# nemo110110/modify-sift-gpu

Hardware: AMD Instinct MI355X
Metric: SIFT images/sec at 1080p (features/sec alongside), 1/2/4/8 MI355X (higher is better)
Workload: dtype f32

## Files before the change

### include/sgpu.h

```cpp
#ifndef SGPU_H
#define SGPU_H
#include <stddef.h>
#include <stdint.h>

#ifdef __cplusplus
extern "C" {
#endif

#define SGPU_OK 0
#define SGPU_EINVAL (-1)
#define SGPU_ENODEV (-2)
#define SGPU_ENOMEM (-3)
#define SGPU_ERANGE (-4)

typedef struct sgpu_options {
    float filter_width_factor;
    float descriptor_window_factor;
    float orientation_window_factor;
    float orientation_gaussian_factor;
    float dog_threshold;
    float edge_threshold;
    int subpixel;
    int max_orientation;
    int fixed_orientation;
// ... 134 lines not shown
#define SGPU_DEBUG_FULL_COLUMNS 128
#define SGPU_DEBUG_DESC_DUAL 256
#define SGPU_DEBUG_ORIENT_WAVE 512
#define SGPU_DEBUG_GAUSS_TILE_ALWAYS 1024
#define SGPU_DEBUG_MATCH_REGSTAGE 2048
#define SGPU_DEBUG_PYR_SERIAL 4096
#define SGPU_DEBUG_GAUSS_LONG_BANDS 8192
#define SGPU_DEBUG_DUO_ALWAYS 16384
#define SGPU_DEBUG_DUO_OFF 32768
#define SGPU_DEBUG_GAUSS_TILE_OFF 65536
#define SGPU_DEBUG_DESC_WIDE_OFF 131072
#define SGPU_DEBUG_DESC_WIDE_ALWAYS 262144
#define SGPU_DEBUG_EXTREMA_TILE_OFF 524288

int sgpu_debug_set_flags(sgpu_ctx* ctx, int flags);
#define SGPU_TRIO_OFF 0
#define SGPU_TRIO_ON 1
#define SGPU_TRIO_ALWAYS 2
#define SGPU_PAIRS_FRONT 0
#define SGPU_PAIRS_END 1
int sgpu_debug_set_schedule(sgpu_ctx* ctx, int trio, int pairs);
#define SGPU_DUO_STRIPS_RULE 0
#define SGPU_DUO_STRIPS_WAVE 1
#define SGPU_DUO_STRIPS_COOP 2
int sgpu_debug_set_duo_strips(sgpu_ctx* ctx, int mode);
int sgpu_debug_set_match_prune(sgpu_ctx* ctx, int on);
int sgpu_debug_match_plan_stats(const sgpu_ctx* ctx, long long out[4]);
#define SGPU_PLAN_ENTRY_INTS 7
#define SGPU_PLAN_LEVEL 0
#define SGPU_PLAN_TILE 1
// ... 17 lines not shown
```

### modify-sift-gpu_amd/csrc/sgpu_capi.cpp

```cpp
#include <dlfcn.h>
#include <hip/hip_runtime.h>
#include <rccl/rccl.h>

#include <algorithm>
#include <cmath>
#include <cstdio>
#include <cstdlib>
#include <atomic>
#include <cstring>
#include <string>
#include <vector>

#include "../../include/sgpu.h"
#include "sift_kernels.h"
#include "sift_match_plan.h"
#include "sift_params.h"
#include "sift_pyramid_plan.h"

namespace {

#ifndef SGK_WIDE_DESC_MAX
#define SGK_WIDE_DESC_MAX 8192
#endif

// ... 81 lines not shown
struct sgpu_ctx {
    int device = 0;
    hipStream_t stream = nullptr;
    sgpu_options opt{};
    sgp::Schedule sched{};
    sgp::InputPlan plan{};
    int debug_flags = 0;
    bool multi_stream = false;
    bool duo_on = false;
    bool duo_wide = false;
    bool duo_u8 = false;
    int trio_mode = SGPU_TRIO_OFF;
    int duo_plan = SGK_DUO_PLAN;
    int duo_strips = SGPU_DUO_STRIPS_RULE;
    size_t wide_desc_max = SGK_WIDE_DESC_MAX;
    bool unit_input = true;
    bool tile_duo = false;
    int tile_mb = SGK_TILE_MB;
    int env_flags = 0;
    struct HostOut {
        float* keys = nullptr;
        float* desc = nullptr;
        int cap = 0;
        bool armed = false, active = false, done = false;
    } host_out;
    bool stage_timing = true;
    bool streaming = false;
    std::string err;
    int batch = 0, w = 0, h = 0, nparts = 0;
    std::vector<sgp::Octave> oct;
    size_t staged_bytes = 0;
    std::vector<int64_t> img_off;
    Part part[kMaxParts];
    DevBuf input, all_keys, all_desc, gray, pre;
// ... 193 lines not shown
    ctx->device = device;
    if (hipSetDevice(device) != hipSuccess ||
        hipStreamCreateWithFlags(&ctx->stream, hipStreamNonBlocking) != hipSuccess) {
        delete ctx;
        return SGPU_ENODEV;
    }
    for (int i = 0; i <= T_N; i++) (void)hipEventCreate(&ctx->ev[i]);
    {
        Part* p = ctx->part;
        bool ok = part_streams(p[0], PS_MAIN) == SGPU_OK && part_streams(p[0], PS_OCT) == SGPU_OK &&
                  hipStreamCreateWithFlags(&ctx->h2d, hipStreamNonBlocking) == hipSuccess &&
                  hipStreamCreateWithFlags(&ctx->d2h, hipStreamNonBlocking) == hipSuccess &&
                  part_streams(p[0], PS_LO) == SGPU_OK && part_streams(p[1], PS_OCT) == SGPU_OK &&
                  part_streams(p[2], PS_MAIN) == SGPU_OK && part_streams(p[2], PS_LO) == SGPU_OK &&
                  part_streams(p[1], PS_MAIN) == SGPU_OK && part_streams(p[1], PS_LO) == SGPU_OK;
        for (int i = 0; ok && i < 2; i++)
            ok = hipEventCreateWithFlags(&ctx->up_ev[i], hipEventDisableTiming) == hipSuccess &&
                 hipEventCreateWithFlags(&ctx->down_ev[i], hipEventDisableTiming) == hipSuccess;
        if (!ok) {
            sgpu_ctx_destroy(ctx);
            return SGPU_ENODEV;
        }
    }
    if (const char* ev = getenv("SGPU_EXACT_DESCRIPTOR"))
        if (ev[0] == '1') ctx->debug_flags |= SGPU_DEBUG_EXACT_DESCRIPTOR;
    if (const char* ev = getenv("SGPU_GAUSS")) {
        if (!strcmp(ev, "block")) ctx->debug_flags |= SGPU_DEBUG_GAUSS_BLOCK;
    }
    if (const char* ev = getenv("SGPU_DUO")) {
        if (!strcmp(ev, "off")) ctx->debug_flags |= SGPU_DEBUG_DUO_OFF;
// ... 22 lines not shown
    }
    if (const char* ev = getenv("SGPU_STREAMS")) ctx->multi_stream = !strcmp(ev, "multi");
    if (const char* ev = getenv("SGPU_MATCH"))
        if (!strcmp(ev, "reg")) ctx->debug_flags |= SGPU_DEBUG_MATCH_REGSTAGE;
    if (const char* ev = getenv("SGPU_DESC")) {
        if (!strcmp(ev, "dual")) ctx->debug_flags |= SGPU_DEBUG_DESC_DUAL;
        if (!strcmp(ev, "narrow")) ctx->debug_flags |= SGPU_DEBUG_DESC_WIDE_OFF;
        if (!strcmp(ev, "wide")) ctx->debug_flags |= SGPU_DEBUG_DESC_WIDE_ALWAYS;
    }
    if (const char* ev = getenv("SGPU_GAUSS_TILE")) {
        if (!strcmp(ev, "off")) ctx->debug_flags |= SGPU_DEBUG_GAUSS_TILE_OFF;
        if (!strcmp(ev, "always")) ctx->debug_flags |= SGPU_DEBUG_GAUSS_TILE_ALWAYS;
    }
    if (const char* ev = getenv("SGPU_WIDE_DESC_MAX"))
        if (atoll(ev) >= 0) ctx->wide_desc_max = (size_t)atoll(ev);
    if (const char* ev = getenv("SGPU_EXTREMA")) {
        if (!strcmp(ev, "wave")) ctx->debug_flags |= SGPU_DEBUG_EXTREMA_TILE_OFF;
    }
    if (const char* ev = getenv("SGPU_TILE_DUO"))
        ctx->tile_duo = !strcmp(ev, "on");
    if (const char* ev = getenv("SGPU_MATCH_PRUNE"))
        ctx->match_prune = strcmp(ev, "off") != 0;
    if (const char* ev = getenv("SGPU_GAUSS_TILE_MB"))
        if (atoi(ev) >= 0) ctx->tile_mb = atoi(ev);
    ctx->env_flags = ctx->debug_flags;
    int rc = sgpu_ctx_set_options(ctx, opt);
    if (rc != SGPU_OK) {
        sgpu_ctx_destroy(ctx);
        return rc;
    }
    *out = ctx;
    return SGPU_OK;
}
// ... 84 lines not shown
    fp.origin_offset = O.lowe_origin ? 0.0f : 0.5f;
    fp.octave_min = ctx->plan.octave_min + ctx->plan.ds;

    const size_t sum_px = (size_t)goff / (size_t)std::max(1, nlev) / (size_t)n;
    pt.cand_cap = (ctx->debug_flags & SGPU_DEBUG_TINY_CAP)
                      ? std::max<size_t>(pt.cand_cap, 64)
                      : std::max(pt.cand_cap, std::max<size_t>(1024, sum_px / 256 * n));
    const size_t nc = pt.cand_cap, ne_cap = 2 * nc;
    ALLOCCHK(ctx, pt.pyr.ensure((size_t)goff * sizeof(float) + 256));
    ALLOCCHK(ctx, pt.mask.ensure((size_t)moff * sizeof(uint32_t)));
    ALLOCCHK(ctx, pt.row_count.ensure((size_t)pt.total_rows * sizeof(uint32_t)));
    ALLOCCHK(ctx, pt.row_base.ensure(((size_t)pt.total_rows + 1) * sizeof(uint32_t)));
    ALLOCCHK(ctx, pt.img_off_dev.ensure((size_t)(n + 2) * sizeof(int64_t)));
    ALLOCCHK(ctx, pt.cand.ensure(nc * sizeof(float4)));
    ALLOCCHK(ctx, pt.info.ensure(nc * sizeof(int2)));
    ALLOCCHK(ctx, pt.ocount.ensure(nc * sizeof(uint32_t)));
    ALLOCCHK(ctx, pt.eoff.ensure((nc + 1) * sizeof(uint32_t)));
    ALLOCCHK(ctx, pt.feat.ensure(ne_cap * sizeof(float4)));
    ALLOCCHK(ctx, pt.feat_info.ensure(ne_cap * sizeof(int2)));
    ALLOCCHK(ctx, pt.keys.ensure(ne_cap * sizeof(float4)));
    if (O.descriptors) ALLOCCHK(ctx, pt.desc.ensure(ne_cap * 128 * sizeof(float)));
    ALLOCCHK(ctx, pt.scan_tmp.ensure((sgk::scan_tmp_words(std::max<size_t>(nc, pt.total_rows)) + 16) * 4));
    if (pt.h_read_n < (size_t)n + 2) {
        if (pt.h_read) (void)hipHostFree(pt.h_read);
        pt.h_read = nullptr;
        g_allocs++;
        ALLOCCHK(ctx, hipHostMalloc((void**)&pt.h_read, ((size_t)n + 2) * sizeof(int64_t)));
        pt.h_read_n = (size_t)n + 2;
    }
    return SGPU_OK;
}
// ... 58 lines not shown
            op.dst = lvl0 + k * od.level_stride;
            op.dst_img_stride = npx;
            op.w = od.wa;
            op.h = od.h;
            op.batch = n;
            op.ds_dst = dk ? ds : nullptr;
            op.ds_w = dk ? dsw : 0;
            op.ds_h = dk ? dsh : 0;
            op.ds_img_stride = dk ? ds_stride : 0;
            if (o == 0 && k == 0 && pt.one_stream) {
                op.zero.p[0] = pt.row_count.as<uint32_t>();
                op.zero.n[0] = (size_t)pt.total_rows;
                op.zero.p[1] = pt.mask.as<uint32_t>();
                op.zero.n[1] = (size_t)pt.mask_words;
                op.zero.p[2] = pt.ocount.as<uint32_t>();
                op.zero.n[2] = pt.cand_cap;
            }
            pt.levels.push_back(sgpyr::LevelDesc{o, k, op.fw, op.w, op.h, op.batch, dk,
                                                 op.src_u8 != nullptr,
                                                 (op.zero.n[0] | op.zero.n[1] | op.zero.n[2]) != 0});
        }
    }
    pt.gauss_filters = (int)pt.ops.size();
    return SGPU_OK;
}

struct OpSupport {
    const sgk::LevelOp* op;
    bool tile(int i) const { return sgk::gauss_tile_supported(op[i]); }
    bool tile_duo(int i, int j) const { return sgk::gauss_tile_duo_supported(op[i], op[j]); }
    bool duo(int i, int j) const { return sgk::gauss_duo_supported(op[i], op[j]); }
// ... 101 lines not shown
    if (O.feature_count_threshold > 0)
        HIPCHK(ctx, sgk::launch_limit_rows(pt.row_count.as<uint32_t>(), fp,
                                           O.feature_count_threshold, O.truncate_method, st));
    HIPCHK(ctx, rec(7, st));
    HIPCHK(ctx, sgk::launch_scan(pt.row_count.as<uint32_t>(), pt.row_base.as<uint32_t>(),
                                 pt.total_rows, pt.scan_tmp.as<uint32_t>(), st));
    HIPCHK(ctx, rec(2, st));

    if (!pt.one_stream) {
        st = pt.stream_lo;
        HIPCHK(ctx, hipStreamWaitEvent(st, pt.ev[2], 0));
    }
    if (wait_lo) HIPCHK(ctx, hipStreamWaitEvent(st, wait_lo, 0));
    const uint32_t* n_cand_dev = pt.row_base.as<uint32_t>() + pt.total_rows;
    if (!pt.one_stream)
        HIPCHK(ctx, sgk::launch_zero(pt.ocount.as<uint32_t>(), nc, nullptr, 0, nullptr, 0, st));
    const int cand_grid = (int)std::min(nc, pt.cand_hint ? pt.cand_hint : nc);
    const bool ori_wave = (ctx->debug_flags & SGPU_DEBUG_ORIENT_WAVE) ||
                          (pt.cand_hint > 0 && pt.cand_hint <= kWaveOrientationMax);
    const int feat_grid = (int)std::min(ne_cap, pt.feat_hint ? pt.feat_hint : ne_cap);
    const bool desc_wide = !(ctx->debug_flags & SGPU_DEBUG_DESC_WIDE_OFF) &&
                           ((ctx->debug_flags & SGPU_DEBUG_DESC_WIDE_ALWAYS) ||
                            (pt.feat_hint > 0 && pt.feat_hint <= ctx->wide_desc_max));
    HIPCHK(ctx, sgk::launch_orientation(pyr, pt.mask.as<uint32_t>(), pt.row_base.as<uint32_t>(),
                                        pt.total_rows, n_cand_dev, (int)nc, cand_grid, fp,
                                        pt.cand.as<float4>(), pt.info.as<int2>(),
                                        pt.ocount.as<uint32_t>(), st, ori_wave));
    if (O.feature_count_threshold > 0 && fp.num_orientation >= 2)
        HIPCHK(ctx, sgk::launch_limit_oriented(pt.ocount.as<uint32_t>(), pt.row_base.as<uint32_t>(),
                                               fp, O.feature_count_threshold, O.truncate_method,
                                               (uint32_t)nc, st));
    HIPCHK(ctx, rec(3, st));
    const uint32_t* n_feat_dev = pt.eoff.as<uint32_t>() + nc;
    sgk::ImageOffsetsArgs io;
    io.row_base = pt.row_base.as<uint32_t>();
    io.batch = n;
    io.rows_per_image = fp.rows_per_image;
    io.total_rows = pt.total_rows;
    io.off = pt.img_off_dev.as<int64_t>();
    HIPCHK(ctx, sgk::launch_scan(pt.ocount.as<uint32_t>(), pt.eoff.as<uint32_t>(), nc,
                                 pt.scan_tmp.as<uint32_t>(), st));
    HIPCHK(ctx, sgk::launch_expand(pt.cand.as<float4>(), pt.info.as<int2>(),
// ... 7 lines not shown
    const bool host_in_desc = pt.copied_out && O.descriptors && desc_wide && !exact_desc && !dual_desc;
    sgk::HostCopy hcopy;
    if (host_in_desc) {
        hcopy.keys = pt.keys.as<float4>();
        hcopy.rec = pt.img_off_dev.as<int64_t>();
        hcopy.rec_n = n + 2;
        hcopy.cap = (uint32_t)ctx->host_out.cap;
        hcopy.hkeys = reinterpret_cast<float4*>(ctx->host_out.keys);
        hcopy.hdesc = ctx->host_out.desc;
        hcopy.hrec = pt.h_read;
    }
    if (O.descriptors)
        HIPCHK(ctx, sgk::launch_descriptor(pyr, pt.feat.as<float4>(), pt.feat_info.as<int2>(),
                                           n_feat_dev, feat_grid, fp, pt.desc.as<float>(), st,
                                           nullptr, false, exact_desc, dual_desc, desc_wide,
                                           host_in_desc ? &hcopy : nullptr));
    HIPCHK(ctx, rec(5, st));
    if (pt.copied_out && !host_in_desc)
        HIPCHK(ctx, sgk::launch_copy_out(pt.keys.as<float4>(), O.descriptors ? pt.desc.as<float>() : nullptr,
                                         n_feat_dev, ctx->host_out.cap, pt.img_off_dev.as<int64_t>(),
                                         n + 2, ctx->host_out.keys,
                                         O.descriptors ? ctx->host_out.desc : nullptr, pt.h_read, st));
    return SGPU_OK;
}

static int enqueue_readback(sgpu_ctx* ctx, Part& pt) {
    hipStream_t st = pt.one_stream ? pt.stream : pt.stream_lo;
    if (!pt.copied_out)
        HIPCHK(ctx, hipMemcpyAsync(pt.h_read, pt.img_off_dev.p, (size_t)(pt.n + 2) * sizeof(int64_t),
                                   hipMemcpyDeviceToHost, st));
    if (pt.events) HIPCHK(ctx, hipEventRecord(pt.ev[6], st));
// ... 1330 lines not shown
            p[1 + 2 * j] = l.op[j] < 0 ? -1 : pt.levels[l.op[j]].o;
            p[2 + 2 * j] = l.op[j] < 0 ? -1 : pt.levels[l.op[j]].k;
        }
    }
    return n;
}

static_assert(SGPU_DUO_STRIPS_RULE == sgk::kDuoStripsRule && SGPU_DUO_STRIPS_WAVE == sgk::kDuoStripsWave &&
              SGPU_DUO_STRIPS_COOP == sgk::kDuoStripsCoop, "sgpu.h and sift_kernels.h agree");
int sgpu_debug_set_duo_strips(sgpu_ctx* ctx, int mode) {
    if (!ctx || mode < SGPU_DUO_STRIPS_RULE || mode > SGPU_DUO_STRIPS_COOP) return SGPU_EINVAL;
    ctx->duo_strips = mode;
    return SGPU_OK;
}

int sgpu_debug_set_schedule(sgpu_ctx* ctx, int trio, int pairs) {
    if (!ctx || trio < SGPU_TRIO_OFF || trio > SGPU_TRIO_ALWAYS || pairs < SGPU_PAIRS_FRONT ||
        pairs > SGPU_PAIRS_END)
        return SGPU_EINVAL;
    ctx->trio_mode = trio;
    ctx->duo_plan = pairs;
    return SGPU_OK;
}

int sgpu_debug_geometry(const sgpu_ctx* ctx, int* n_octaves, int* dims, int max) {
    if (!ctx || !n_octaves) return SGPU_EINVAL;
    *n_octaves = (int)ctx->oct.size();
    for (int o = 0; o < (int)ctx->oct.size() && o < max; o++) {
        dims[3 * o] = ctx->oct[o].w;
        dims[3 * o + 1] = ctx->oct[o].h;
// ... 74 lines not shown
```

### modify-sift-gpu_amd/csrc/sift_kernels.h

```cpp
#pragma once
#include <hip/hip_runtime.h>
#include <stdint.h>

namespace sgk {

constexpr int kMaxLevels = 16;
constexpr int kMaxOctaves = 16;

struct Taps { float k[33]; };

struct OctaveDesc {
    int w, h, wa;
    int nwords;
    long long gauss_off;
    long long level_stride;
    long long mask_off;
    long long mask_level_stride;
};

struct FeatureParams {
    int batch, n_octaves, d;
    int rows_per_image;
    int row_off[kMaxOctaves];
    float level_sigma[kMaxLevels];
// ... 65 lines not shown
                                     int dw, int dh, long long dst_img_stride, int batch,
                                     hipStream_t stream);

hipError_t launch_color_to_gray(const uint8_t* src, int n, int w, int h, int stride,
                                int channels, bool bgr, float* dst, hipStream_t stream);

hipError_t launch_extrema(const float* pyr, uint32_t* mask, uint32_t* row_count,
                          const FeatureParams& fp, hipStream_t stream, bool tiles = false);

size_t scan_tmp_words(size_t n);
hipError_t launch_zero(uint32_t* a, size_t na, uint32_t* b, size_t nb, uint32_t* c, size_t nc,
                       hipStream_t stream);
hipError_t launch_scan(const uint32_t* in, uint32_t* out, size_t n, uint32_t* tmp,
                       hipStream_t stream);

hipError_t launch_orientation(const float* pyr, const uint32_t* mask, const uint32_t* row_base,
                              int total_rows, const uint32_t* n_cand_dev, int n_cand_cap,
                              int grid_hint, const FeatureParams& fp, float4* out4, int2* info,
                              uint32_t* ocount, hipStream_t stream,
                              bool wave_per_candidate = false);

struct ImageOffsetsArgs {
    const uint32_t* row_base = nullptr;
    int batch = 0, rows_per_image = 0, total_rows = 0;
    int64_t* off = nullptr;
};
hipError_t launch_expand(const float4* cand, const int2* info, const uint32_t* eoff,
                         const uint32_t* n_cand_dev, int n_cand_cap, const FeatureParams& fp,
                         float4* feat, int2* feat_info, float4* keys, hipStream_t stream,
                         const ImageOffsetsArgs* io = nullptr);

hipError_t launch_copy_out(const float4* keys, const float* desc, const uint32_t* n_dev, int cap,
                           const int64_t* rec, int rec_n, float* hkeys, float* hdesc,
                           int64_t* hrec, hipStream_t stream);

struct HostCopy {
    const float4* keys = nullptr;
    const int64_t* rec = nullptr;
    int rec_n = 0;
    uint32_t cap = 0;
    float4* hkeys = nullptr;
    float* hdesc = nullptr;
    int64_t* hrec = nullptr;
};
hipError_t launch_descriptor(const float* pyr, const float4* feat, const int2* feat_info,
                             const uint32_t* n_feat_dev, int n_feat_cap, const FeatureParams& fp,
                             float* desc, hipStream_t stream, const int* out_index = nullptr,
                             bool rect = false, bool exact = false, bool dual = false,
                             bool wide = false, const HostCopy* host = nullptr);

hipError_t launch_orient_keys(const float* pyr, float4* feat, const int2* feat_info,
                              const int* index, int n, const FeatureParams& fp, float4* keys_out,
                              hipStream_t stream);

hipError_t launch_limit_rows(uint32_t* row_count, const FeatureParams& fp, int threshold,
                             int method, hipStream_t stream);
hipError_t launch_limit_oriented(uint32_t* ocount, const uint32_t* row_base,
                                 const FeatureParams& fp, int threshold, int method,
                                 uint32_t cand_cap, hipStream_t stream);


typedef hipError_t (*DebugCandidatesFn)(const float* pyr, const uint32_t* mask,
                                        const uint32_t* row_base, int total_rows,
                                        const uint32_t* n_cand_dev, int n_cand_cap,
// ... 74 lines not shown
```

### modify-sift-gpu_amd/csrc/sift_kernels.hip

```cpp
#include <cstdlib>
#include <cstring>
#include <numeric>
#include <type_traits>
#include <utility>

#include "sift_kernels.h"
#include "sift_math.h"

using namespace sgm;

#include "sift_keys.h"

namespace sgk {
namespace {

__device__ __forceinline__ int clampi(int v, int lo, int hi) { return v < lo ? lo : (v > hi ? hi : v); }

constexpr int GT = 64;
typedef float f2v __attribute__((ext_vector_type(2)));

__device__ __forceinline__ f2v pk_fma(f2v a, float b, f2v c) {
    return __builtin_elementwise_fma(a, f2v{b, b}, c);
}

// ... 1374 lines not shown
__global__ __launch_bounds__(256) void k_orientation(const float* __restrict__ pyr,
                                                     const uint32_t* __restrict__ mask,
                                                     const uint32_t* __restrict__ row_base,
                                                     int total_rows,
                                                     const uint32_t* __restrict__ n_cand_dev,
                                                     uint32_t cap, const FeatureParams fp,
                                                     float4* __restrict__ out4,
                                                     int2* __restrict__ info,
                                                     uint32_t* __restrict__ ocount) {
    __shared__ float s_vote[64 * 37];
    const int sub = threadIdx.x & 3, slot = threadIdx.x >> 2;
    const uint32_t n = min(*n_cand_dev, cap);
    float* vote_l = s_vote + slot * 37;
    for (uint32_t f = blockIdx.x * 64 + slot; f < n; f += gridDim.x * 64)
        orientation_one(f, sub, vote_l, pyr, mask, row_base, total_rows, fp, out4, info, ocount);
}

template <bool U8>
__device__ __forceinline__ float input_at(const float* sf, const uint8_t* s8, int stride, int tw,
                                          int h, long long k) {
    if (k >= (long long)tw * h) return 0.0f;
    const int r = (int)(k / tw), c = (int)(k - (long long)r * tw);
    return U8 ? u8_to_unit(s8[(long long)r * stride + c]) : sf[(long long)r * stride + c];
}

template <bool U8>
__global__ __launch_bounds__(256) void k_input_down(const float* __restrict__ src,
                                                    const uint8_t* __restrict__ src8, int stride,
                                                    long long src_img_stride, int tw, int h,
                                                    int fo, float* __restrict__ dst, int dw, int dh,
// ... 1058 lines not shown
                                                         const float4* __restrict__ feat,
                                                         const int2* __restrict__ feat_info,
                                                         const uint32_t* __restrict__ n_feat_dev,
                                                         const FeatureParams fp,
                                                         float* __restrict__ desc,
                                                         const int* __restrict__ out_index) {
    __shared__ __attribute__((aligned(16))) float s_flat[4][kFlatWords];
    const int lane = threadIdx.x & 63;
    const uint32_t wave = __builtin_amdgcn_readfirstlane(threadIdx.x >> 6);
    const uint32_t n = *n_feat_dev;
    for (uint32_t e = blockIdx.x * 4 + wave; e < n; e += gridDim.x * 4)
        descriptor_flat(e, lane, pyr, feat, feat_info, fp, desc,
                        out_index ? (uint32_t)out_index[e] : e, s_flat[wave]);
}

template <int NWV>
__global__ __launch_bounds__(64 * NWV) SGK_FLAT_ATTR void k_descriptor_wide(const float* __restrict__ pyr,
                                                         const float4* __restrict__ feat,
                                                         const int2* __restrict__ feat_info,
                                                         const uint32_t* __restrict__ n_feat_dev,
                                                         const FeatureParams fp,
                                                         float* __restrict__ desc,
                                                         const int* __restrict__ out_index,
                                                         const HostCopy hc) {
    __shared__ __attribute__((aligned(16))) float s_flat[NWV][kFlatWords];
    const int lane = threadIdx.x & 63;
    const int wave = __builtin_amdgcn_readfirstlane(threadIdx.x >> 6);
    const uint32_t n = *n_feat_dev;
    if (hc.hrec && blockIdx.x == 0 && threadIdx.x < (unsigned)hc.rec_n) hc.hrec[threadIdx.x] = hc.rec[threadIdx.x];
    for (uint32_t e = blockIdx.x; e < n; e += gridDim.x) {
// ... 399 lines not shown
    }
    if (n <= 32768) {
        hipLaunchKernelGGL(k_scan_single, dim3(1), dim3(1024), 0, stream, in, out, n);
        return hipGetLastError();
    }
    const size_t nb = scan_blocks(n);
    uint32_t* sums = tmp;
    uint32_t* sums_scan = tmp + nb;
    hipLaunchKernelGGL(k_scan_block, dim3((unsigned)nb), dim3(256), 0, stream, in, out, n, sums);
    hipError_t e = launch_scan(sums, sums_scan, nb, tmp + nb + nb + 1, stream);
    if (e != hipSuccess) return e;
    hipLaunchKernelGGL(k_scan_add, dim3((unsigned)nb), dim3(256), 0, stream, out, n, sums_scan);
    return hipGetLastError();
}

hipError_t launch_orientation(const float* pyr, const uint32_t* mask, const uint32_t* row_base,
                              int total_rows, const uint32_t* n_cand_dev, int n_cand_cap,
                              int grid_hint, const FeatureParams& fp, float4* out4, int2* info,
                              uint32_t* ocount, hipStream_t stream, bool wave_per_candidate) {
    if (n_cand_cap <= 0) return hipSuccess;
    if (wave_per_candidate) {
        const unsigned grid = (unsigned)std::max(1LL, std::min(((long long)grid_hint + 3) / 4, 8192LL));
        hipLaunchKernelGGL(k_orientation_wave, dim3(grid), dim3(256), 0, stream, pyr, mask,
                           row_base, total_rows, n_cand_dev, (uint32_t)n_cand_cap, fp, out4, info,
                           ocount);
        return hipGetLastError();
    }
    const unsigned grid = (unsigned)std::max(1LL, std::min(((long long)grid_hint + 63) / 64, 4096LL));
    hipLaunchKernelGGL(k_orientation, dim3(grid), dim3(256), 0, stream, pyr, mask, row_base,
                       total_rows, n_cand_dev, (uint32_t)n_cand_cap, fp, out4, info, ocount);
    return hipGetLastError();
}

__global__ __launch_bounds__(256) void k_copy_out(const float4* __restrict__ keys,
                                                  const float4* __restrict__ desc,
// ... 36 lines not shown
}

hipError_t launch_orient_keys(const float* pyr, float4* feat, const int2* feat_info,
                              const int* index, int n, const FeatureParams& fp, float4* keys_out,
                              hipStream_t stream) {
    if (n <= 0) return hipSuccess;
    const unsigned grid = (unsigned)std::min((n + 63) / 64, 4096);
    hipLaunchKernelGGL(k_orient_keys, dim3(grid), dim3(256), 0, stream, pyr, feat, feat_info,
                       index, n, fp, keys_out);
    return hipGetLastError();
}

hipError_t launch_descriptor(const float* pyr, const float4* feat, const int2* feat_info,
                             const uint32_t* n_feat_dev, int n_feat_cap, const FeatureParams& fp,
                             float* desc, hipStream_t stream, const int* out_index,
                             bool rect, bool exact, bool dual, bool wide, const HostCopy* host) {
    if (n_feat_cap <= 0) return hipSuccess;
    if (host && (!wide || exact || rect || dual || host->rec_n < 0 || host->rec_n > 256 ||
                 !host->hkeys || !host->hrec || !host->keys || !host->rec))
        return hipErrorInvalidValue;
    const unsigned grid = (unsigned)std::min(((long long)n_feat_cap + 3) / 4, 65536LL);
#ifndef SGK_DESC_DUAL
#define SGK_DESC_DUAL 1
#endif
#ifndef SGK_DESC_FLAT
#define SGK_DESC_FLAT 1
#endif
    if (!exact && !rect && SGK_DESC_FLAT && !dual && wide) {
        static const int nwv = [] {
            const char* e = getenv("SGPU_WIDE_DESC_WAVES");
            return e && atoi(e) == 8 ? 8 : 4;
        }();
        static const long long gmax = [] {
            const char* e = getenv("SGPU_WIDE_DESC_GRID");
            return e && atoll(e) > 0 ? atoll(e) : 65536LL;
        }();
        const unsigned wgrid = (unsigned)std::min((long long)n_feat_cap, gmax);
        const HostCopy hc = host ? *host : HostCopy{};
        if (nwv == 8)
            hipLaunchKernelGGL(k_descriptor_wide<8>, dim3(wgrid), dim3(512), 0, stream, pyr, feat,
                               feat_info, n_feat_dev, fp, desc, out_index, hc);
        else
            hipLaunchKernelGGL(k_descriptor_wide<4>, dim3(wgrid), dim3(256), 0, stream, pyr, feat,
                               feat_info, n_feat_dev, fp, desc, out_index, hc);
        return hipGetLastError();
    }
    if (!exact && !rect && SGK_DESC_FLAT && !dual) {
        hipLaunchKernelGGL(k_descriptor_flat, dim3(grid), dim3(256), 0, stream, pyr, feat,
                           feat_info, n_feat_dev, fp, desc, out_index);
        return hipGetLastError();
    }
    if (!exact && !rect && SGK_DESC_DUAL) {
        hipLaunchKernelGGL(k_descriptor_dual, dim3(grid), dim3(256), 0, stream, pyr, feat,
                           feat_info, n_feat_dev, fp, desc, out_index);
        return hipGetLastError();
    }
    if (!exact) {
        if (rect)
            hipLaunchKernelGGL(k_descriptor_fast<true>, dim3(grid), dim3(256), 0, stream, pyr,
                               feat, feat_info, n_feat_dev, fp, desc, out_index);
        else
// ... 33 lines not shown
```

### modify-sift-gpu_amd/python/sgpu.py

```python
from __future__ import annotations

import contextlib
import ctypes
import os
import subprocess

import numpy as np

from sgpu_types import SgpuOptions, default_options

PKG = os.path.dirname(os.path.dirname(os.path.abspath(__file__)))
LIB_PATH = os.environ.get("SGPU_LIB_PATH") or os.path.join(PKG, "lib", "libsiftgpu.so")

SGPU_OK, SGPU_EINVAL, SGPU_ENODEV, SGPU_ENOMEM, SGPU_ERANGE = 0, -1, -2, -3, -4
SGPU_INPUT_HOST, SGPU_INPUT_DEVICE, SGPU_INPUT_STAGED = 0, 1, 2

C_API = [
    "sgpu_default_options", "sgpu_parse_args", "sgpu_ctx_create", "sgpu_ctx_destroy",
    "sgpu_ctx_set_options", "sgpu_last_error", "sgpu_device_count", "sgpu_extract",
    "sgpu_extract_f32", "sgpu_stage_input", "sgpu_feature_count", "sgpu_feature_total", "sgpu_copy_features",
    "sgpu_device_features", "sgpu_match", "sgpu_quantize_descriptors", "sgpu_last_timing",
    "sgpu_debug_geometry", "sgpu_debug_gaussian", "sgpu_debug_candidates",
    "sgpu_debug_set_flags", "sgpu_comm_unique_id", "sgpu_comm_init", "sgpu_comm_allgather_i32",
    "sgpu_comm_allreduce_f64", "sgpu_extract_keypoints", "sgpu_match_guided", "sgpu_extract_color",
    "sgpu_match_shard_begin", "sgpu_match_shard_end", "sgpu_match_sharded",
    "sgpu_extract_stream", "sgpu_host_alloc", "sgpu_host_free", "sgpu_reserve",
    "sgpu_debug_alloc_count", "sgpu_last_pyramid_launches", "sgpu_set_stage_timing",
    "sgpu_set_host_output", "sgpu_debug_set_schedule", "sgpu_debug_set_match_prune",
    "sgpu_quantize_descriptors_gpu", "sgpu_feature_descriptors_u8", "sgpu_copy_features_u8",
    "sgpu_match_batch", "sgpu_match_images", "sgpu_debug_match_plan_stats",
    "sgpu_debug_set_duo_strips", "sgpu_debug_pyramid_plan",
    "sgpu_match_batch_guided", "sgpu_match_images_guided",
]

PLAN_KINDS = ("level", "tile", "two", "tile_two", "tile_duo", "tile_duo_one", "duo", "trio")

_LIB = None


def build():
    subprocess.check_call(["make", "-C", PKG, "-j8"])


def lib():
    global _LIB
    if _LIB is None:
# ... 23 lines not shown
        L.sgpu_feature_total.restype = c.c_int64
        L.sgpu_copy_features.argtypes = [vp, c.c_int, vp, vp]
        L.sgpu_device_features.argtypes = [vp, P(vp), P(vp), P(vp)]
        L.sgpu_match.argtypes = [vp, vp, c.c_int, vp, c.c_int, c.c_float, c.c_float, c.c_int,
                                 c.c_int, vp, c.c_int]
        L.sgpu_match_guided.argtypes = [vp, vp, c.c_int, vp, c.c_int, vp, vp, vp, vp, c.c_float,
                                        c.c_float, c.c_float, c.c_float, c.c_int, c.c_int, vp,
                                        c.c_int]
        L.sgpu_extract_color.argtypes = [vp, vp, c.c_int, c.c_int, c.c_int, c.c_int, c.c_int, c.c_int]
        L.sgpu_quantize_descriptors.argtypes = [vp, c.c_size_t, vp]
        L.sgpu_last_timing.argtypes = [vp, vp, c.c_int]
        L.sgpu_debug_set_flags.argtypes = [vp, c.c_int]
        L.sgpu_debug_set_schedule.argtypes = [vp, c.c_int, c.c_int]
        L.sgpu_debug_set_match_prune.argtypes = [vp, c.c_int]
        L.sgpu_debug_set_duo_strips.argtypes = [vp, c.c_int]
        L.sgpu_debug_geometry.argtypes = [vp, P(c.c_int), vp, c.c_int]
        L.sgpu_debug_gaussian.argtypes = [vp, c.c_int, c.c_int, c.c_int, vp]
        L.sgpu_debug_candidates.argtypes = [vp, vp, vp, c.c_int, P(c.c_int)]
        L.sgpu_extract_keypoints.argtypes = [vp, c.c_int, vp, c.c_int, c.c_int]
        L.sgpu_comm_unique_id.argtypes = [vp, c.c_int]
        L.sgpu_comm_init.argtypes = [vp, c.c_int, c.c_int, vp, c.c_int]
        L.sgpu_comm_allgather_i32.argtypes = [vp, vp, c.c_int, vp]
        L.sgpu_comm_allreduce_f64.argtypes = [vp, vp, c.c_int, c.c_int]
        L.sgpu_match_shard_begin.argtypes = [vp, vp, c.c_int, c.c_int, vp, c.c_int, c.c_float,
                                             c.c_float, c.c_int, vp, vp, c.c_int]
        L.sgpu_match_shard_end.argtypes = [vp, c.c_int, c.c_int, vp, c.c_int, c.c_int, c.c_float,
                                           c.c_float, c.c_int, c.c_int, vp]
        L.sgpu_match_sharded.argtypes = [vp, vp, c.c_int, c.c_int, vp, c.c_int, c.c_float,
                                         c.c_float, c.c_int, c.c_int, vp, c.c_int]
        L.sgpu_extract_stream.argtypes = [vp, P(vp), c.c_int, c.c_int, c.c_int, c.c_int, c.c_int,
# ... 498 lines not shown

    def set_debug_flags(self, flags: int):
        self._check(lib().sgpu_debug_set_flags(self._ctx, flags), "sgpu_debug_set_flags")

    TRIO_OFF, TRIO_ON, TRIO_ALWAYS = 0, 1, 2
    PAIRS_FRONT, PAIRS_END = 0, 1

    def set_schedule(self, trio: int = 0, pairs: int = 1):
        self._check(lib().sgpu_debug_set_schedule(self._ctx, trio, pairs), "sgpu_debug_set_schedule")

    STRIPS_RULE, STRIPS_WAVE, STRIPS_COOP = 0, 1, 2

    def set_duo_strips(self, mode: int = 0):
        self._check(lib().sgpu_debug_set_duo_strips(self._ctx, mode), "sgpu_debug_set_duo_strips")

    def set_match_prune(self, on: bool = True):
        self._check(lib().sgpu_debug_set_match_prune(self._ctx, int(bool(on))),
                    "sgpu_debug_set_match_prune")

    def match_plan_stats(self):
        out = np.zeros(4, np.int64)
        self._check(lib().sgpu_debug_match_plan_stats(self._ctx, out.ctypes.data),
                    "sgpu_debug_match_plan_stats")
        return dict(zip(["items", "sides", "max_tiles", "max_chunks"], out.tolist()))

    @contextlib.contextmanager
    def exact_descriptors(self):
        self.set_debug_flags(self.DEBUG_EXACT_DESCRIPTOR)
        try:
            yield self
# ... 25 lines not shown
```

Baseline: 18520.

## Add atomic work-queue persistent kernels for orientation and descriptor stages

Orientation and descriptor kernels are replaced by persistent, occupancy-sized grids. Each wave pulls work units from striped atomic counters placed after the ocount buffer, so the grid adapts to the device-side candidate and feature counts instead of using a static grid-stride assignment. The aim is better load balance and fewer idle or over-launched blocks when the counts vary. The cost is atomic traffic, extra buffer zeroing, and a dependence on occupancy queries made at context creation. The feature is on by default and can be switched off through an environment variable or a debug API.

New measurement: 18840, median of 6. +1.8%, better.

```diff
diff --git a/include/sgpu.h b/include/sgpu.h
--- a/include/sgpu.h
+++ b/include/sgpu.h
@@ -172,6 +172,11 @@
 #define SGPU_DEBUG_EXTREMA_TILE_OFF 524288
 
 int sgpu_debug_set_flags(sgpu_ctx* ctx, int flags);
+#define SGPU_FEATURES_QUEUE 0
+#define SGPU_FEATURES_STATIC_ORIENTATION 1
+#define SGPU_FEATURES_STATIC_DESCRIPTOR 2
+#define SGPU_FEATURES_STATIC 3
+int sgpu_debug_set_feature_queue(sgpu_ctx* ctx, int mode);
 #define SGPU_TRIO_OFF 0
 #define SGPU_TRIO_ON 1
 #define SGPU_TRIO_ALWAYS 2
diff --git a/modify-sift-gpu_amd/csrc/sgpu_capi.cpp b/modify-sift-gpu_amd/csrc/sgpu_capi.cpp
--- a/modify-sift-gpu_amd/csrc/sgpu_capi.cpp
+++ b/modify-sift-gpu_amd/csrc/sgpu_capi.cpp
@@ -119,10 +119,13 @@
     int duo_plan = SGK_DUO_PLAN;
     int duo_strips = SGPU_DUO_STRIPS_RULE;
     size_t wide_desc_max = SGK_WIDE_DESC_MAX;
+    size_t wave_orient_max = kWaveOrientationMax;
     bool unit_input = true;
     bool tile_duo = false;
     int tile_mb = SGK_TILE_MB;
     int env_flags = 0;
+    sgk::FeatureQueue fq{};
+    bool queue_ori = true, queue_desc = true;
     struct HostOut {
         float* keys = nullptr;
         float* desc = nullptr;
@@ -346,6 +349,7 @@
                   part_streams(p[0], PS_LO) == SGPU_OK && part_streams(p[1], PS_OCT) == SGPU_OK &&
                   part_streams(p[2], PS_MAIN) == SGPU_OK && part_streams(p[2], PS_LO) == SGPU_OK &&
                   part_streams(p[1], PS_MAIN) == SGPU_OK && part_streams(p[1], PS_LO) == SGPU_OK;
+        ok = ok && sgk::feature_queue_grids(&ctx->fq) == hipSuccess;
         for (int i = 0; ok && i < 2; i++)
             ok = hipEventCreateWithFlags(&ctx->up_ev[i], hipEventDisableTiming) == hipSuccess &&
                  hipEventCreateWithFlags(&ctx->down_ev[i], hipEventDisableTiming) == hipSuccess;
@@ -398,9 +402,22 @@
     }
     if (const char* ev = getenv("SGPU_WIDE_DESC_MAX"))
         if (atoll(ev) >= 0) ctx->wide_desc_max = (size_t)atoll(ev);
+    if (const char* ev = getenv("SGPU_WAVE_ORIENT_MAX"))
+        if (atoll(ev) >= 0) ctx->wave_orient_max = (size_t)atoll(ev);
     if (const char* ev = getenv("SGPU_EXTREMA")) {
         if (!strcmp(ev, "wave")) ctx->debug_flags |= SGPU_DEBUG_EXTREMA_TILE_OFF;
     }
+    if (const char* ev = getenv("SGPU_FEATURE_QUEUE")) {
+        if (!strcmp(ev, "on") || !strcmp(ev, "ori") || !strcmp(ev, "desc") || !strcmp(ev, "off")) {
+            ctx->queue_ori = !strcmp(ev, "on") || !strcmp(ev, "ori");
+            ctx->queue_desc = !strcmp(ev, "on") || !strcmp(ev, "desc");
+        }
+    }
+    if (const char* ev = getenv("SGPU_FEATURE_QUEUE_GRID"))
+        if (atoi(ev) >= 1) {
+            ctx->fq.ori_grid = std::min(ctx->fq.ori_grid, atoi(ev));
+            ctx->fq.desc_grid = std::min(ctx->fq.desc_grid, atoi(ev));
+        }
     if (const char* ev = getenv("SGPU_TILE_DUO"))
         ctx->tile_duo = !strcmp(ev, "on");
     if (const char* ev = getenv("SGPU_MATCH_PRUNE"))
@@ -515,7 +532,7 @@
     ALLOCCHK(ctx, pt.img_off_dev.ensure((size_t)(n + 2) * sizeof(int64_t)));
     ALLOCCHK(ctx, pt.cand.ensure(nc * sizeof(float4)));
     ALLOCCHK(ctx, pt.info.ensure(nc * sizeof(int2)));
-    ALLOCCHK(ctx, pt.ocount.ensure(nc * sizeof(uint32_t)));
+    ALLOCCHK(ctx, pt.ocount.ensure((sgk::feature_queue_base(nc) + sgk::kFeatureQueueWords) * sizeof(uint32_t)));
     ALLOCCHK(ctx, pt.eoff.ensure((nc + 1) * sizeof(uint32_t)));
     ALLOCCHK(ctx, pt.feat.ensure(ne_cap * sizeof(float4)));
     ALLOCCHK(ctx, pt.feat_info.ensure(ne_cap * sizeof(int2)));
@@ -604,7 +621,7 @@
                 op.zero.p[1] = pt.mask.as<uint32_t>();
                 op.zero.n[1] = (size_t)pt.mask_words;
                 op.zero.p[2] = pt.ocount.as<uint32_t>();
-                op.zero.n[2] = pt.cand_cap;
+                op.zero.n[2] = sgk::feature_queue_base(pt.cand_cap) + sgk::kFeatureQueueWords;
             }
             pt.levels.push_back(sgpyr::LevelDesc{o, k, op.fw, op.w, op.h, op.batch, dk,
                                                  op.src_u8 != nullptr,
@@ -736,10 +753,13 @@
     if (wait_lo) HIPCHK(ctx, hipStreamWaitEvent(st, wait_lo, 0));
     const uint32_t* n_cand_dev = pt.row_base.as<uint32_t>() + pt.total_rows;
     if (!pt.one_stream)
-        HIPCHK(ctx, sgk::launch_zero(pt.ocount.as<uint32_t>(), nc, nullptr, 0, nullptr, 0, st));
+        HIPCHK(ctx, sgk::launch_zero(pt.ocount.as<uint32_t>(), sgk::feature_queue_base(nc) + sgk::kFeatureQueueWords,
+                                     nullptr, 0, nullptr, 0, st));
+    sgk::FeatureQueue fq = ctx->fq;
+    fq.next = pt.ocount.as<uint32_t>() + sgk::feature_queue_base(nc);
     const int cand_grid = (int)std::min(nc, pt.cand_hint ? pt.cand_hint : nc);
     const bool ori_wave = (ctx->debug_flags & SGPU_DEBUG_ORIENT_WAVE) ||
-                          (pt.cand_hint > 0 && pt.cand_hint <= kWaveOrientationMax);
+                          (pt.cand_hint > 0 && pt.cand_hint <= ctx->wave_orient_max);
     const int feat_grid = (int)std::min(ne_cap, pt.feat_hint ? pt.feat_hint : ne_cap);
     const bool desc_wide = !(ctx->debug_flags & SGPU_DEBUG_DESC_WIDE_OFF) &&
                            ((ctx->debug_flags & SGPU_DEBUG_DESC_WIDE_ALWAYS) ||
@@ -747,7 +767,8 @@
     HIPCHK(ctx, sgk::launch_orientation(pyr, pt.mask.as<uint32_t>(), pt.row_base.as<uint32_t>(),
                                         pt.total_rows, n_cand_dev, (int)nc, cand_grid, fp,
                                         pt.cand.as<float4>(), pt.info.as<int2>(),
-                                        pt.ocount.as<uint32_t>(), st, ori_wave));
+                                        pt.ocount.as<uint32_t>(), st, ori_wave,
+                                        ctx->queue_ori ? &fq : nullptr));
     if (O.feature_count_threshold > 0 && fp.num_orientation >= 2)
         HIPCHK(ctx, sgk::launch_limit_oriented(pt.ocount.as<uint32_t>(), pt.row_base.as<uint32_t>(),
                                                fp, O.feature_count_threshold, O.truncate_method,
@@ -785,7 +806,8 @@
         HIPCHK(ctx, sgk::launch_descriptor(pyr, pt.feat.as<float4>(), pt.feat_info.as<int2>(),
                                            n_feat_dev, feat_grid, fp, pt.desc.as<float>(), st,
                                            nullptr, false, exact_desc, dual_desc, desc_wide,
-                                           host_in_desc ? &hcopy : nullptr));
+                                           host_in_desc ? &hcopy : nullptr,
+                                           ctx->queue_desc ? &fq : nullptr));
     HIPCHK(ctx, rec(5, st));
     if (pt.copied_out && !host_in_desc)
         HIPCHK(ctx, sgk::launch_copy_out(pt.keys.as<float4>(), O.descriptors ? pt.desc.as<float>() : nullptr,
@@ -2146,6 +2168,13 @@
     return SGPU_OK;
 }
 
+int sgpu_debug_set_feature_queue(sgpu_ctx* ctx, int mode) {
+    if (!ctx || mode < SGPU_FEATURES_QUEUE || mode > SGPU_FEATURES_STATIC) return SGPU_EINVAL;
+    ctx->queue_ori = !(mode & SGPU_FEATURES_STATIC_ORIENTATION);
+    ctx->queue_desc = !(mode & SGPU_FEATURES_STATIC_DESCRIPTOR);
+    return SGPU_OK;
+}
+
 int sgpu_debug_set_schedule(sgpu_ctx* ctx, int trio, int pairs) {
     if (!ctx || trio < SGPU_TRIO_OFF || trio > SGPU_TRIO_ALWAYS || pairs < SGPU_PAIRS_FRONT ||
         pairs > SGPU_PAIRS_END)
diff --git a/modify-sift-gpu_amd/csrc/sift_kernels.h b/modify-sift-gpu_amd/csrc/sift_kernels.h
--- a/modify-sift-gpu_amd/csrc/sift_kernels.h
+++ b/modify-sift-gpu_amd/csrc/sift_kernels.h
@@ -103,11 +103,26 @@
 hipError_t launch_scan(const uint32_t* in, uint32_t* out, size_t n, uint32_t* tmp,
                        hipStream_t stream);
 
+constexpr int kQueueCounters = 8;
+constexpr int kQueueStride = 32;
+constexpr size_t kFeatureQueueWords = 2 * kQueueCounters * kQueueStride;
+constexpr size_t feature_queue_base(size_t n_cand_cap) {
+    return (n_cand_cap + kQueueStride - 1) / kQueueStride * kQueueStride;
+}
+struct FeatureQueue {
+    uint32_t* next = nullptr;
+    int ori_grid = 0;
+    int desc_grid = 0;
+    int desc_waves = 1;
+};
+hipError_t feature_queue_grids(FeatureQueue* q);
+
 hipError_t launch_orientation(const float* pyr, const uint32_t* mask, const uint32_t* row_base,
                               int total_rows, const uint32_t* n_cand_dev, int n_cand_cap,
                               int grid_hint, const FeatureParams& fp, float4* out4, int2* info,
                               uint32_t* ocount, hipStream_t stream,
-                              bool wave_per_candidate = false);
+                              bool wave_per_candidate = false,
+                              const FeatureQueue* queue = nullptr);
 
 struct ImageOffsetsArgs {
     const uint32_t* row_base = nullptr;
@@ -136,7 +151,8 @@
                              const uint32_t* n_feat_dev, int n_feat_cap, const FeatureParams& fp,
                              float* desc, hipStream_t stream, const int* out_index = nullptr,
                              bool rect = false, bool exact = false, bool dual = false,
-                             bool wide = false, const HostCopy* host = nullptr);
+                             bool wide = false, const HostCopy* host = nullptr,
+                             const FeatureQueue* queue = nullptr);
 
 hipError_t launch_orient_keys(const float* pyr, float4* feat, const int2* feat_info,
                               const int* index, int n, const FeatureParams& fp, float4* keys_out,
diff --git a/modify-sift-gpu_amd/csrc/sift_kernels.hip b/modify-sift-gpu_amd/csrc/sift_kernels.hip
--- a/modify-sift-gpu_amd/csrc/sift_kernels.hip
+++ b/modify-sift-gpu_amd/csrc/sift_kernels.hip
@@ -1412,6 +1412,40 @@
     float* vote_l = s_vote + slot * 37;
     for (uint32_t f = blockIdx.x * 64 + slot; f < n; f += gridDim.x * 64)
         orientation_one(f, sub, vote_l, pyr, mask, row_base, total_rows, fp, out4, info, ocount);
+}
+
+__device__ __forceinline__ uint32_t queue_ask(uint32_t* next, uint32_t wave) {
+    uint32_t i = 0;
+    if ((threadIdx.x & 63) == 0)
+        i = __hip_atomic_fetch_add(next + (wave % kQueueCounters) * kQueueStride, 1u,
+                                   __ATOMIC_RELAXED, __HIP_MEMORY_SCOPE_AGENT);
+    return i;
+}
+__device__ __forceinline__ uint32_t queue_unit(uint32_t ticket, uint32_t wave, uint32_t nwaves) {
+    return nwaves + __builtin_amdgcn_readfirstlane(ticket) * kQueueCounters + wave % kQueueCounters;
+}
+
+__global__ __launch_bounds__(64) void k_orientation_queue(const float* __restrict__ pyr,
+                                                          const uint32_t* __restrict__ mask,
+                                                          const uint32_t* __restrict__ row_base,
+                                                          int total_rows,
+                                                          const uint32_t* __restrict__ n_cand_dev,
+                                                          uint32_t cap, const FeatureParams fp,
+                                                          float4* __restrict__ out4,
+                                                          int2* __restrict__ info,
+                                                          uint32_t* __restrict__ ocount,
+                                                          uint32_t* __restrict__ next) {
+    __shared__ float s_vote[16 * 37];
+    const int sub = threadIdx.x & 3, slot = threadIdx.x >> 2;
+    const uint32_t n = min(*n_cand_dev, cap);
+    const uint32_t groups = (n + 15) / 16;
+    float* vote_l = s_vote + slot * 37;
+    for (uint32_t g = blockIdx.x; g < groups;
+         g = queue_unit(queue_ask(next, blockIdx.x), blockIdx.x, gridDim.x)) {
+        const uint32_t f = 16 * g + slot;
+        if (f < n)
+            orientation_one(f, sub, vote_l, pyr, mask, row_base, total_rows, fp, out4, info, ocount);
+    }
 }
 
 template <bool U8>
@@ -2500,6 +2534,28 @@
                         out_index ? (uint32_t)out_index[e] : e, s_flat[wave]);
 }
 
+template <int NW>
+__global__ __launch_bounds__(64 * NW) SGK_FLAT_ATTR void k_descriptor_queue(
+    const float* __restrict__ pyr, const float4* __restrict__ feat,
+    const int2* __restrict__ feat_info, const uint32_t* __restrict__ n_feat_dev,
+    const FeatureParams fp, float* __restrict__ desc, const int* __restrict__ out_index,
+    uint32_t* __restrict__ next) {
+    __shared__ __attribute__((aligned(16))) float s_flat[NW][kFlatWords];
+    const int lane = threadIdx.x & 63;
+    const uint32_t wave = NW == 1 ? 0u : __builtin_amdgcn_readfirstlane(threadIdx.x >> 6);
+    float* sh = s_flat[wave];
+    const uint32_t n = *n_feat_dev;
+    const uint32_t wv = blockIdx.x * NW + wave, nwaves = gridDim.x * NW;
+    for (uint32_t e = wv; e < n;) {
+        flat_accumulate(e, lane, pyr, feat, feat_info, fp, sh, 0, 1);
+        const uint32_t out = out_index ? (uint32_t)out_index[e] : e;
+        const bool narrow = flat_narrow(fp, flat_half_box(feat[e], fp));
+        const uint32_t ticket = queue_ask(next, wv);
+        flat_finish(lane, fp, desc, out, sh, 1, narrow);
+        e = queue_unit(ticket, wv, nwaves);
+    }
+}
+
 template <int NWV>
 __global__ __launch_bounds__(64 * NWV) SGK_FLAT_ATTR void k_descriptor_wide(const float* __restrict__ pyr,
                                                          const float4* __restrict__ feat,
@@ -2929,11 +2985,36 @@
     return hipGetLastError();
 }
 
+hipError_t feature_queue_grids(FeatureQueue* q) {
+    int dev = 0, cus = 0, ori = 0, d1 = 0, d2 = 0;
+    hipError_t e = hipGetDevice(&dev);
+    if (e == hipSuccess) e = hipDeviceGetAttribute(&cus, hipDeviceAttributeMultiprocessorCount, dev);
+    if (e == hipSuccess) e = hipOccupancyMaxActiveBlocksPerMultiprocessor(&ori, k_orientation_queue, 64, 0);
+    if (e == hipSuccess) e = hipOccupancyMaxActiveBlocksPerMultiprocessor(&d1, k_descriptor_queue<1>, 64, 0);
+    if (e == hipSuccess) e = hipOccupancyMaxActiveBlocksPerMultiprocessor(&d2, k_descriptor_queue<2>, 128, 0);
+    if (e != hipSuccess) return e;
+    if (cus <= 0 || ori <= 0 || d1 <= 0 || d2 <= 0) return hipErrorInvalidValue;
+    q->desc_waves = 2 * d2 > d1 ? 2 : 1;
+    q->ori_grid = ori * cus;
+    q->desc_grid = (q->desc_waves == 2 ? d2 : d1) * cus;
+    return hipSuccess;
+}
+
 hipError_t launch_orientation(const float* pyr, const uint32_t* mask, const uint32_t* row_base,
                               int total_rows, const uint32_t* n_cand_dev, int n_cand_cap,
                               int grid_hint, const FeatureParams& fp, float4* out4, int2* info,
-                              uint32_t* ocount, hipStream_t stream, bool wave_per_candidate) {
+                              uint32_t* ocount, hipStream_t stream, bool wave_per_candidate,
+                              const FeatureQueue* queue) {
     if (n_cand_cap <= 0) return hipSuccess;
+    if (queue && !wave_per_candidate) {
+        if (!queue->next || queue->ori_grid <= 0) return hipErrorInvalidValue;
+        const long long groups = ((long long)n_cand_cap + 15) / 16;
+        const unsigned grid = (unsigned)std::max<long long>(kQueueCounters, std::min<long long>(groups, queue->ori_grid));
+        hipLaunchKernelGGL(k_orientation_queue, dim3(grid), dim3(64), 0, stream, pyr, mask,
+                           row_base, total_rows, n_cand_dev, (uint32_t)n_cand_cap, fp, out4, info,
+                           ocount, queue->next);
+        return hipGetLastError();
+    }
     if (wave_per_candidate) {
         const unsigned grid = (unsigned)std::max(1LL, std::min(((long long)grid_hint + 3) / 4, 8192LL));
         hipLaunchKernelGGL(k_orientation_wave, dim3(grid), dim3(256), 0, stream, pyr, mask,
@@ -3000,7 +3081,8 @@
 hipError_t launch_descriptor(const float* pyr, const float4* feat, const int2* feat_info,
                              const uint32_t* n_feat_dev, int n_feat_cap, const FeatureParams& fp,
                              float* desc, hipStream_t stream, const int* out_index,
-                             bool rect, bool exact, bool dual, bool wide, const HostCopy* host) {
+                             bool rect, bool exact, bool dual, bool wide, const HostCopy* host,
+                             const FeatureQueue* queue) {
     if (n_feat_cap <= 0) return hipSuccess;
     if (host && (!wide || exact || rect || dual || host->rec_n < 0 || host->rec_n > 256 ||
                  !host->hkeys || !host->hrec || !host->keys || !host->rec))
@@ -3031,6 +3113,20 @@
                                feat_info, n_feat_dev, fp, desc, out_index, hc);
         return hipGetLastError();
     }
+    if (!exact && !rect && SGK_DESC_FLAT && !dual && queue) {
+        const int nw = queue->desc_waves;
+        if (!queue->next || queue->desc_grid <= 0 || (nw != 1 && nw != 2)) return hipErrorInvalidValue;
+        uint32_t* qa = queue->next + kQueueCounters * kQueueStride;
+        const long long wgs = ((long long)n_feat_cap + nw - 1) / nw;
+        const unsigned qgrid = (unsigned)std::max<long long>(kQueueCounters, std::min<long long>(wgs, queue->desc_grid));
+        if (nw == 2)
+            hipLaunchKernelGGL(k_descriptor_queue<2>, dim3(qgrid), dim3(128), 0, stream, pyr, feat,
+                               feat_info, n_feat_dev, fp, desc, out_index, qa);
+        else
+            hipLaunchKernelGGL(k_descriptor_queue<1>, dim3(qgrid), dim3(64), 0, stream, pyr, feat,
+                               feat_info, n_feat_dev, fp, desc, out_index, qa);
+        return hipGetLastError();
+    }
     if (!exact && !rect && SGK_DESC_FLAT && !dual) {
         hipLaunchKernelGGL(k_descriptor_flat, dim3(grid), dim3(256), 0, stream, pyr, feat,
                            feat_info, n_feat_dev, fp, desc, out_index);
diff --git a/modify-sift-gpu_amd/python/sgpu.py b/modify-sift-gpu_amd/python/sgpu.py
--- a/modify-sift-gpu_amd/python/sgpu.py
+++ b/modify-sift-gpu_amd/python/sgpu.py
@@ -29,7 +29,7 @@
     "sgpu_set_host_output", "sgpu_debug_set_schedule", "sgpu_debug_set_match_prune",
     "sgpu_quantize_descriptors_gpu", "sgpu_feature_descriptors_u8", "sgpu_copy_features_u8",
     "sgpu_match_batch", "sgpu_match_images", "sgpu_debug_match_plan_stats",
-    "sgpu_debug_set_duo_strips", "sgpu_debug_pyramid_plan",
+    "sgpu_debug_set_duo_strips", "sgpu_debug_pyramid_plan", "sgpu_debug_set_feature_queue",
     "sgpu_match_batch_guided", "sgpu_match_images_guided",
 ]
 
@@ -83,6 +83,7 @@
         L.sgpu_debug_set_schedule.argtypes = [vp, c.c_int, c.c_int]
         L.sgpu_debug_set_match_prune.argtypes = [vp, c.c_int]
         L.sgpu_debug_set_duo_strips.argtypes = [vp, c.c_int]
+        L.sgpu_debug_set_feature_queue.argtypes = [vp, c.c_int]
         L.sgpu_debug_geometry.argtypes = [vp, P(c.c_int), vp, c.c_int]
         L.sgpu_debug_gaussian.argtypes = [vp, c.c_int, c.c_int, c.c_int, vp]
         L.sgpu_debug_candidates.argtypes = [vp, vp, vp, c.c_int, P(c.c_int)]
@@ -611,6 +612,11 @@
     def set_duo_strips(self, mode: int = 0):
         self._check(lib().sgpu_debug_set_duo_strips(self._ctx, mode), "sgpu_debug_set_duo_strips")
 
+    FEATURES_QUEUE, FEATURES_STATIC_ORIENTATION, FEATURES_STATIC_DESCRIPTOR, FEATURES_STATIC = 0, 1, 2, 3
+
+    def set_feature_queue(self, mode: int = 0):
+        self._check(lib().sgpu_debug_set_feature_queue(self._ctx, mode), "sgpu_debug_set_feature_queue")
+
     def set_match_prune(self, on: bool = True):
         self._check(lib().sgpu_debug_set_match_prune(self._ctx, int(bool(on))),
                     "sgpu_debug_set_match_prune")
```
